# XuyangBai/PointDSC

Hardware: AMD Instinct MI355X
Metric: point-cloud pairs/sec @ N=5000 corr (higher is better)
Workload: dtype f32 (attention products as fp16x3 split (fp16 hi+lo operand pairs, three f16 MFMAs per product), f32 accumulate; fc_message / PointCN products as fp16 hi+lo split; spatial-consistency matrix stored as unorm16); 1 GPU; 3DMatch-like synthetic correspondences (BASELINE.json configs[2]): N=5000 corr, 32 pairs per step sharded over 1 GPU(s) = 32 per GPU, 12-layer PointDSC, seeded random weights; num_corr=5000, pairs_per_gpu=32, global_batch=32, compat_format=u16, layer_gemm=h3, att_leaves=canonical, latency_mode=False, range_guard=lazy (pipeline), collective=none (single process, no process group)

## Files before the change

include/pointdsc_hip.h:

```cpp
#ifndef POINTDSC_HIP_H
#define POINTDSC_HIP_H

#include <stddef.h>

#ifdef __cplusplus
extern "C" {
#endif

#define PDSC_VERSION 10
#define PDSC_CHANNELS 128
#define PDSC_MAX_K 64
#define PDSC_MAX_POWER_ITERS 32

enum pdsc_status {
    PDSC_OK = 0,
    PDSC_ERR_ARG = -1,
    PDSC_ERR_WORKSPACE = -2,
    PDSC_ERR_LAUNCH = -3
};

typedef struct pdsc_config {
    int in_dim;
    int num_layers;
    int num_channels;
// ... 92 lines not shown
    const float* part_ml;
    int nsplit, Npad;
    const float* res;
    const float* feat_in;
    float* feat_out;
    float* featB_out;
    float* qkv_out;
    void* q_split;
    void* kv_tiles;
    const void* w1; const float* b1;
    const void* w2; const float* b2;
    const void* w3; const float* b3;
    const void* wp; const float* bp;
    const void* wq; const float* bq;
    const void* wq_split;
    const void* wfrag_tail;
    const void* wfrag_head;
    int gemm_format;
    int io_flags;
    int bs, N;
    int kernel;
} pdsc_layer_call;
int pdsc_layer_run(const pdsc_layer_call* call, void* stream);

size_t    pdsc_wsplit_bytes(const pdsc_config* cfg);
long long pdsc_wsplit_offset(const pdsc_config* cfg, int section, int layer);
int       pdsc_wsplit_build(const pdsc_config* cfg, const float* wpack, void* wsplit, void* stream);
#define PDSC_WS_FRAG_TAIL 100
#define PDSC_WS_FRAG_HEAD 101
#define PDSC_WS_FRAG_TAIL_H3 102
#define PDSC_WS_FRAG_HEAD_H3 103
#define PDSC_WS_FOLD_TAIL_H3 104
#define PDSC_WS_FOLD_HEAD_H3 105
#define PDSC_WS_FOLD_W 106
size_t pdsc_wfrag_fold_tail_bytes(void);
size_t pdsc_wfrag_fold_head_bytes(void);
int pdsc_layer_prefers_block(int bs, int N);
int pdsc_layer_h3_uses_coop(int bs, int N);
size_t pdsc_wfrag_tail_bytes(void);
size_t pdsc_wfrag_head_bytes(void);
int pdsc_wfrag_build_tail(const float* w1, const float* b1, const float* w2, const float* b2, const float* w3,
                          const float* b3, void* out, int gemm_format, void* stream);
int pdsc_wfrag_build_head(const float* wp, const float* bp, const float* wq, const float* bq, void* out,
                          int gemm_format, void* stream);

size_t pdsc_attention_scratch_bytes(int bs, int N, int nsplit);
// ... 300 lines not shown
```

pointdsc_amd/_lib.py:

```python
from __future__ import annotations

import ctypes as C
import os
from pathlib import Path

PKG = Path(__file__).resolve().parent
LIB_PATH = Path(os.environ.get("POINTDSC_HIP_LIB", PKG / "libpointdsc_hip.so"))


class PointDSCLibraryError(RuntimeError):
    pass


class PdscConfig(C.Structure):
    _fields_ = [
        ("in_dim", C.c_int), ("num_layers", C.c_int), ("num_channels", C.c_int),
        ("num_iterations", C.c_int), ("k", C.c_int), ("refine_iters", C.c_int),
        ("inlier_threshold", C.c_float), ("nms_radius", C.c_float), ("refine_threshold", C.c_float),
        ("attention_precision", C.c_int), ("compat_format", C.c_int), ("layer_gemm", C.c_int),
        ("att_leaves", C.c_int), ("value_fold", C.c_int),
    ]


W_SECTIONS = [
# ... 25 lines not shown
        [("workspace", _vp), ("workspace_bytes", _sz), ("num_corr", _vp), ("num_seeds_per_pair", _vp), ("n_min", _i)] +
        [(n, _vp) for n in ("tail_stream", "fork_event", "join_event", "absmax", "range_report")])


ABI_VERSION = 10

SIGNATURES = {
    "pdsc_version": (_i, []),
    "pdsc_last_error": (C.c_char_p, []),
    "pdsc_experiments_enabled": (_i, []),
    "pdsc_wpack_floats": (_ll, [_cfgp]),
    "pdsc_wpack_offset": (_ll, [_cfgp, _i, _i]),
    "pdsc_compat_ld": (_ll, [_i]),
    "pdsc_workspace_bytes": (_sz, [_cfgp, _i, _i, _i]),
    "pdsc_workspace_offset": (_ll, [_cfgp, _i, _i, _i, C.c_char_p]),
    "pdsc_spatial_compat": (_i, [_vp, _vp, _vp, _vp, _vp, _ll, _i, _i, _vp]),
    "pdsc_spatial_compat_u16": (_i, [_vp, _vp, _vp, _vp, _ll, _i, _i, _vp]),
    "pdsc_selftest_exact_math": (_i, [_vp, _f, _vp, _vp, _ll, _vp]),
    "pdsc_selftest_mfma_valu_neighbour": (_i, [_vp, _i, _i, _vp]),
    "pdsc_classifier_hidden": (_i, [_vp, _vp, _vp, _vp, _vp, _vp, _i, _vp]),
    "pdsc_linear": (_i, [_vp, _ll, _vp, _vp, _vp, _ll, _vp, _ll, _i, _i, _i, _i, _vp]),
    "pdsc_layer0": (_i, [_vp, _i, _vp, _vp, _vp, _i, _vp]),
    "pdsc_layer_run": (_i, [C.POINTER(PdscLayerCall), _vp]),
    "pdsc_wsplit_bytes": (_sz, [_cfgp]),
    "pdsc_wsplit_offset": (_ll, [_cfgp, _i, _i]),
    "pdsc_wsplit_build": (_i, [_cfgp, _vp, _vp, _vp]),
    "pdsc_layer_prefers_block": (_i, [_i, _i]),
    "pdsc_layer_h3_uses_coop": (_i, [_i, _i]),
    "pdsc_wfrag_tail_bytes": (_sz, []),
    "pdsc_wfrag_head_bytes": (_sz, []),
    "pdsc_wfrag_fold_tail_bytes": (_sz, []),
    "pdsc_wfrag_fold_head_bytes": (_sz, []),
    "pdsc_wfrag_build_tail": (_i, [_vp] * 7 + [_i, _vp]),
    "pdsc_wfrag_build_head": (_i, [_vp] * 5 + [_i, _vp]),
    "pdsc_sc_attention_split_partials": (_i, [_vp, _vp, _vp, _i, _ll, _vp, _sz, _i, _i, _i, _i, _vp]),
    "pdsc_split_q_bytes": (_sz, [_i, _i]),
    "pdsc_split_kv_bytes": (_sz, [_i, _i]),
    "pdsc_pack_qkv_split": (_i, [_vp, _vp, _vp, _i, _i, _vp]),
    "pdsc_attention_split_scratch_bytes": (_sz, [_i, _i, _i]),
    "pdsc_attention_split_default_split": (_i, [_i, _i]),
    "pdsc_attention_leaf_count": (_i, [_i]),
    "pdsc_attention_leaf_plan": (_i, [_i, _i, _i, C.POINTER(C.c_int), C.POINTER(C.c_int)]),
    "pdsc_attention_leaf_scratch_bytes": (_sz, [_i, _i, _i]),
    "pdsc_attention_trace": (_i, [_vp]),
    "pdsc_attention_leaf_split_override": (_i, [_i]),
    "pdsc_layer_trace": (_i, [_vp]),
# ... 137 lines not shown
```

pointdsc_amd/csrc/layer.hip:

```cpp
#include <stdlib.h>
#include <type_traits>
#include "pdsc_common.h"
#include "split_layout.h"
#include "merge_partials.h"
#include "layer_args.h"
#include "layer_block.h"

namespace pdsc {

constexpr int LF_ROWS = 32;
constexpr int LF_LD = PDSC_CHANNELS + 4;
constexpr int LF_TILE = LF_ROWS * LF_LD;


#define LF_STAMP(k)                                                                                   \
    if (a.trace && lane == 0) a.trace[(((size_t)blockIdx.y * gridDim.x + blockIdx.x) * 4 + wave) * 16 + (k)] = __builtin_readcyclecounter();

template <int K>
__device__ __forceinline__ void load_w(const float* __restrict__ W, int n0, int l31, int h, f32x4 (&w)[K / 8]) {
    const float* p = W + (size_t)(n0 + l31) * K + 4 * h;
#pragma unroll
    for (int q = 0; q < K / 8; ++q) w[q] = *reinterpret_cast<const f32x4*>(p + 8 * q);
}

// ... 333 lines not shown
    using pdsc::LayerKernel;
    switch (c.kernel) {
        case PDSC_LAYER_KERNEL_BLOCK: *kernel = LayerKernel::Block; return true;
        case PDSC_LAYER_KERNEL_WAVE: *kernel = LayerKernel::Wave; return true;
        case PDSC_LAYER_KERNEL_H3: *kernel = LayerKernel::H3; return true;
        case PDSC_LAYER_KERNEL_X3: *kernel = LayerKernel::X3; return true;
        case PDSC_LAYER_KERNEL_AUTO: break;
        default: return false;
    }
    if (!a.wf_tail && !a.wf_head) {
        const char* ev = pdsc::env_str("PDSC_LAYER_VARIANT");
        const bool block = ev && (ev[0] == 'b' || ev[0] == 'w') ? ev[0] == 'b' : pdsc_layer_prefers_block(c.bs, c.N) != 0;
        *kernel = block ? LayerKernel::Block : LayerKernel::Wave;
    } else if (c.io_flags != 0) {
        *kernel = LayerKernel::H3;
    } else {
        const bool h3 = c.gemm_format == PDSC_LAYER_GEMM_H3 && pdsc::env_int("PDSC_LAYER_H3_VARIANT", 1) != 0 &&
                        pdsc::launch_layer_h3_fits(a, a.msg != nullptr || a.part_o != nullptr, a.featB_out != nullptr);
        *kernel = h3 ? LayerKernel::H3 : LayerKernel::Wave;
    }
    return true;
}

extern "C" int pdsc_layer_run(const pdsc_layer_call* call, void* stream) {
    PDSC_REQUIRE(call, "pdsc_layer_run: null call");
    const pdsc_layer_call& c = *call;
    const bool natural = c.w1 || c.b1 || c.w2 || c.b2 || c.w3 || c.b3 || c.wp || c.bp || c.wq || c.bq || c.wq_split;
    PDSC_REQUIRE(!natural || (!c.wfrag_tail && !c.wfrag_head), "pdsc_layer_run: weights given in natural layout AND as fragment streams");
    if (c.featB_out && !c.q_split && !c.kv_tiles) PDSC_REQUIRE(c.qkv_out, "pdsc_layer_run: head needs qkv_out when no split streams are given");
    pdsc::LayerArgs a = pdsc::layer_args_from_call(c);
    a.trace = c.io_flags ? nullptr : g_layer_trace;
    pdsc::LayerKernel kernel;
    PDSC_REQUIRE(choose_layer_kernel(c, a, &kernel), "pdsc_layer_run: kernel=%d", c.kernel);
    const int rc = pdsc::validate_layer_args(a, kernel, "pdsc_layer_run");
    return rc != PDSC_OK ? rc : pdsc::dispatch_layer(a, kernel, (hipStream_t)stream);
}
```

pointdsc_amd/csrc/layer_h3.hip:

```cpp
#include <stdlib.h>
#include <type_traits>
#include "pdsc_common.h"
#include "split_layout.h"
#include "merge_partials.h"
#include "layer_args.h"
#include "layer_wave.h"

namespace pdsc {

constexpr int PDSC_H3_COOP_TILES = 2560;

#define LH_STAMP(k) \
    if (TRACE && lane == 0) a.trace[(size_t)gw * 64 + (k)] = __builtin_readcyclecounter();

template <bool F = false>
constexpr int stage_tiles(int stage) { return stage == ST_FC1 || stage == ST_FC2 ? 2 : stage == ST_FC3 || stage == ST_PCN ? 4 : F ? 10 : 12; }

template <bool T, bool H, bool TRACE = false, int PIPE = 6, int EXP = 0, bool FB_PF = false, int NWV = LW_WAVES, int NBUF = 2, bool F = false>
__global__ __launch_bounds__(64 * NWV, NBUF > 2 ? 1 : 2) void layer_h3_kernel(LayerArgs a) {
    __shared__ __attribute__((aligned(16))) float Vs_all[NWV][32 * LW_VLD];
    const int lane = threadIdx.x & 63;
    const int wave = __builtin_amdgcn_readfirstlane(threadIdx.x >> 6);
    const int l31 = lane & 31, h = lane >> 5;
    const int tpp = ceil_div_dev(a.N, 32);
    const int gw = blockIdx.x * NWV + wave;
    if (gw >= a.bs * tpp) return;
    const int b = gw / tpp, tile = gw - b * tpp;
    const int m0 = b * a.N + tile * 32;
    const int valid = min(32, (a.nvalid ? a.nvalid[b] : a.N) - tile * 32);
    if (valid <= 0) return;
    const bool live = l31 < valid;
    const size_t row = (size_t)m0 + min(l31, valid - 1);
    float* Vs = Vs_all[wave];
    unsigned char* patch = reinterpret_cast<unsigned char*>(Vs);

    if (a.stagger_cycles > 0 && blockIdx.x < 512) {
        unsigned hwid;
        asm volatile("s_getreg_b32 %0, hwreg(HW_REG_HW_ID)" : "=s"(hwid));
        const bool late = a.stagger_mode == 1 ? (hwid & 1u) : a.stagger_mode == 2 ? (blockIdx.x & 1) : ((blockIdx.x >> 8) & 1);
        if (late) {
            const long long t0 = __builtin_readcyclecounter();
            while (__builtin_readcyclecounter() - t0 < a.stagger_cycles) __builtin_amdgcn_s_sleep(32);
        }
    }
    LH_STAMP(0)
    float rmax = 0.f;
    constexpr int NCH = num_chunks<T, H, F>();
    constexpr int VW = F ? LW_FOLD_VW : PDSC_CHANNELS;
    constexpr int NQ = VW / 8;
    WChunk w[NBUF];
    static_for<0, NBUF - 1>([&](auto jc) {
        constexpr int j = decltype(jc)::value;
        if constexpr (j < NCH) load_chunk<T, true, true, F>(w[j], a, j, lane);
    });

    u32x4 a0h[8], a0l[8], a1h[4], a1l[4], a2h[4], a2l[4], ayh[8], ayl[8], xqh[8], xql[8];
    f32x4 y3[16];
    if (T) {
        f32x4 x0[16];
        auto first_operand = [&](int kk) __attribute__((always_inline)) {
            if constexpr (F) {
                const float* bpr = reinterpret_cast<const float*>(a.wf_tail + LW_FOLD_BPRIME_BYTES);
#pragma unroll
                for (int u = 0; u < 2; ++u) {
                    const f32x4 bv = *reinterpret_cast<const f32x4*>(bpr + 8 * (2 * kk + u) + 4 * h);
#pragma unroll
                    for (int e = 0; e < 4; ++e) x0[2 * kk + u][e] = fmaxf(x0[2 * kk + u][e] + bv[e], 0.f);
                }
                make_kstep<true>(x0[2 * kk], x0[2 * kk + 1], a1h[kk], a1l[kk], rmax);
            } else {
                make_kstep<true>(x0[2 * kk], x0[2 * kk + 1], a0h[kk], a0l[kk], rmax);
            }
        };
        if (a.msg) {
#pragma unroll
            for (int q = 0; q < NQ; ++q) x0[q] = *reinterpret_cast<const f32x4*>(a.msg + row * VW + 8 * q + 4 * h);
#pragma unroll
// ... 17 lines not shown
                            pv[q][sp] = (EXP & 4) ? f32x4{1.f, 2.f, 3.f, (float)lane}
                                                  : *reinterpret_cast<const f32x4*>(a.part_o + e0 + (size_t)sp * a.Npad * VW + eq * (q0 + q));
#pragma unroll
                    for (int q = 0; q < GQ; ++q) {
#pragma unroll
                        for (int e = 0; e < 4; ++e) {
                            x0[q0 + q][e] = merge_apply<NS>(pv[q], mw, e);
                            asm volatile("" : "+v"(x0[q0 + q][e]));
                        }
                    }
#pragma unroll
                    for (int kk = q0 / 2; kk < (q0 + GQ) / 2; ++kk) first_operand(kk);
                    __builtin_amdgcn_sched_barrier(0);
                }
            });
        }
    } else {
#pragma unroll
        for (int q = 0; q < 16; ++q) y3[q] = *reinterpret_cast<const f32x4*>(a.feat_in + row * PDSC_CHANNELS + 8 * q + 4 * h);
#pragma unroll
        for (int kk = 0; kk < 8; ++kk) make_kstep<true>(y3[2 * kk], y3[2 * kk + 1], ayh[kk], ayl[kk], rmax);
    }
    LH_STAMP(1)

    unsigned char* img = H ? a.kv + (size_t)gw * SPL_TILE_STRIDE : nullptr;
    f32x16 acc, cross;
    f32x4 vp[4];
    u32x4 ev = {0u, 0u, 0u, 0u};
    float vt[8];

    auto epi = [&](auto stage_c, auto tile_c, auto sc, f32x4 (&v)[4]) {
        constexpr ChunkDesc d = {decltype(stage_c)::value, decltype(tile_c)::value, 0, 0};
        constexpr int s = decltype(sc)::value;
        constexpr int n0 = 32 * d.tile;
        if constexpr (d.stage == ST_FC1 || d.stage == ST_FC2) {
            if constexpr (s < 4) {
#pragma unroll
                for (int e = 0; e < 4; ++e) v[s][e] = fmaxf(v[s][e], 0.f);
                if constexpr (s & 1)
                    make_kstep<true>(v[s - 1], v[s], (d.stage == ST_FC1 ? a1h : a2h)[2 * d.tile + (s >> 1)],
                                     (d.stage == ST_FC1 ? a1l : a2l)[2 * d.tile + (s >> 1)], rmax);
            }
        } else if constexpr (d.stage == ST_FC3) {
            if constexpr (s < 4) {
#pragma unroll
                for (int e = 0; e < 4; ++e) y3[4 * d.tile + s][e] = y3[4 * d.tile + s][e] + v[s][e];
// ... 43 lines not shown
                        if constexpr (!(EXP & (2 | 8))) *reinterpret_cast<u32x4*>(dst) = ev;
                        else asm volatile("" :: "v"(ev), "v"(dst));
                    }
                    if constexpr (s >= 3 && s < 7) ev = patch_line(patch, lane, s - 3);
                } else {
                    if constexpr (s < 4) vt_put(Vs, lane, s, zero_unless(live, v[s]));
                    if constexpr (s == 3) wave_lds_sync();
                    if constexpr (s == 4 || s == 6) vt_gather(Vs, lane, (s - 4) >> 1, vt);
                    if constexpr (s == 5 || s == 7) {
                        u32x4 ch, cl;
                        vt_split(vt, ch, cl);
                        const int off = vt_offset<VW>(lane, (s - 5) >> 1, 32 * (d.tile - 8));
                        if constexpr (!(EXP & (2 | 32))) vt_store<VW>(img, off, ch, cl);
                        else asm volatile("" :: "v"(ch), "v"(cl), "v"(off));
                    }
                }
            }
        }
    };

    static_for<0, NCH>([&](auto ic) {
        constexpr int i = decltype(ic)::value;
        constexpr ChunkDesc d = chunk_desc<T, F>(i);
        if constexpr (i + NBUF - 1 < NCH && !((EXP & 1) && i >= 1)) load_chunk<T, true, true, F>(w[(i + NBUF - 1) % NBUF], a, i + NBUF - 1, lane);
        if constexpr (T && d.stage == ST_FC2 && d.tile == 0 && !(EXP & 4)) {
            const bool pf = a.io_flags & PDSC_IO_RES_PF;
            const float* r0 = a.res + (pf ? (size_t)gw * PF_TILE_FLOATS + lane * 4 : row * PDSC_CHANNELS + 4 * h);
            const int eq = pf ? 256 : 8;
#pragma unroll
            for (int q = 0; q < 16; ++q) y3[q] = *reinterpret_cast<const f32x4*>(r0 + eq * q);
        }
        const WChunk& wc = w[i % NBUF];
        if constexpr (d.chunk == 0) acc = bias_step(wc);
        constexpr bool pending = d.tile > 0;
        using StageC = std::integral_constant<int, d.stage>;
        using PrevC = std::integral_constant<int, d.tile - 1>;
        static_for<0, 4>([&](auto gc) {
            constexpr int g = decltype(gc)::value;
            if constexpr (d.stage == ST_QKV) {
                const sp16x8 wh = __builtin_bit_cast(sp16x8, wc.v[2 * g]), wl = __builtin_bit_cast(sp16x8, wc.v[2 * g + 1]);
                const sp16x8 bh = __builtin_bit_cast(sp16x8, xqh[4 * d.chunk + g]), bl = __builtin_bit_cast(sp16x8, xql[4 * d.chunk + g]);
                acc = PDSC_MFMA_X3(wl, bh, acc, 0, 0, 0);
                acc = PDSC_MFMA_X3(wh, bl, acc, 0, 0, 0);
                acc = PDSC_MFMA_X3(wh, bh, acc, 0, 0, 0);
            } else {
                const u32x4* oh = d.stage == ST_FC1 ? a0h : d.stage == ST_FC2 ? a1h : d.stage == ST_FC3 ? a2h : ayh;
                const u32x4* ol = d.stage == ST_FC1 ? a0l : d.stage == ST_FC2 ? a1l : d.stage == ST_FC3 ? a2l : ayl;
                const f32x16 zero = {0.f, 0.f, 0.f, 0.f, 0.f, 0.f, 0.f, 0.f, 0.f, 0.f, 0.f, 0.f, 0.f, 0.f, 0.f, 0.f};
                const f16x8 wh = __builtin_bit_cast(f16x8, wc.v[2 * g]), wl = __builtin_bit_cast(f16x8, wc.v[2 * g + 1]);
                const f16x8 bh = __builtin_bit_cast(f16x8, oh[4 * d.chunk + g]), bl = __builtin_bit_cast(f16x8, ol[4 * d.chunk + g]);
                cross = __builtin_amdgcn_mfma_f32_32x32x16_f16(wl, bh, (d.chunk == 0 && g == 0) ? zero : cross, 0, 0, 0);
                acc = __builtin_amdgcn_mfma_f32_32x32x16_f16(wh, bh, acc, 0, 0, 0);
                cross = __builtin_amdgcn_mfma_f32_32x32x16_f16(wh, bl, cross, 0, 0, 0);
            }
            if constexpr (pending) {
                if constexpr (d.nchunks == 2) {
                    epi(StageC{}, PrevC{}, std::integral_constant<int, 4 * d.chunk + g>{}, vp);
                } else {
                    epi(StageC{}, PrevC{}, std::integral_constant<int, 2 * g>{}, vp);
                    epi(StageC{}, PrevC{}, std::integral_constant<int, 2 * g + 1>{}, vp);
                }
            }
        });
        if constexpr (d.chunk == d.nchunks - 1) {
#pragma unroll
            for (int g = 0; g < 4; ++g)
#pragma unroll
                for (int e = 0; e < 4; ++e) vp[g][e] = d.stage != ST_QKV ? fmaf(cross[4 * g + e], H3_INV, acc[4 * g + e]) : acc[4 * g + e];
            if constexpr (d.tile == stage_tiles<F>(d.stage) - 1) {
                static_for<0, 8>([&](auto sc) { epi(StageC{}, std::integral_constant<int, d.tile>{}, sc, vp); });
            }
        }
// ... 11 lines not shown
    LH_STAMP(63)
    range_report(a.range_flag, b, rmax);
}

bool launch_layer_h3_fits(const LayerArgs& a, bool tail, bool head) {
    if (a.gemm_format != PDSC_LAYER_GEMM_H3) return false;
    if (head && (!a.qs || !a.kv || a.qkv_out)) return false;
    if (tail && head && a.feat_out) return false;
    if (tail && !head && !a.feat_out) return false;
    return a.wf_tail || !tail;
}

H3Form layer_h3_form(const LayerArgs& a, bool tail, bool head) {
    const bool fb_pf = a.io_flags & PDSC_IO_FEATB_PF;
    if (a.value_fold) {
        if (tail && head && fb_pf) return H3Form::FoldTailHeadPF;
        if (head && !tail && fb_pf) return H3Form::FoldHeadPF;
        if (tail && !head) return H3Form::FoldTail;
        set_error("pdsc_layer_run(h3): the folded layer exists with point-fragment featB only");
        return H3Form::Unserved;
    }
    if (head && fb_pf) return tail ? H3Form::TailHeadPF : H3Form::HeadPF;
    return tail && head ? H3Form::TailHead : tail ? H3Form::Tail : H3Form::Head;
}

static void h3_launch_shape(int tiles, int* nwv, int* nbuf) {
    *nwv = LW_WAVES; *nbuf = 2;
    (void)tiles;
#ifdef PDSC_EXPERIMENTS
    const int force = env_int("PDSC_LAYER_H3_SHAPE", 0);
    if (force == 42 || force == 23 || force == 13 || force == 24 || force == 14 || force == 22) { *nwv = force / 10; *nbuf = force % 10; }
#endif
}

int launch_layer_h3(const LayerArgs& a, bool tail, bool head, hipStream_t st) {
    const int waves = a.bs * ceil_div(a.N, 32);
    int nwv, nbuf;
    h3_launch_shape(waves, &nwv, &nbuf);
    if (a.value_fold) { nwv = LW_WAVES; nbuf = 2; }
    const dim3 grid(ceil_div(waves, nwv)), block(64 * nwv);
    const H3Form form = layer_h3_form(a, tail, head);
    if (form == H3Form::Unserved) return PDSC_ERR_ARG;
    const bool timed = tail && head;
    int coop_tiles = PDSC_H3_COOP_TILES;
#ifdef PDSC_EXPERIMENTS
    coop_tiles = env_int("PDSC_LAYER_H3_COOP", coop_tiles);
#endif
    if (waves <= coop_tiles && !a.trace) {
        if (timed) profile_mark_begin(PDSC_PROF_LAYER, st);
        const int rc = launch_layer_h3_coop(a, tail, head, st);
        if (timed) profile_mark_end(PDSC_PROF_LAYER, st);
        return rc;
    }
    if (timed) profile_mark_begin(PDSC_PROF_LAYER, st);
#ifdef PDSC_EXPERIMENTS
#define PDSC_H3_LAUNCH_EXTRA(TT, HH, PF)                                                                                            \
        if (nwv == 1 && nbuf == 4) hipLaunchKernelGGL((layer_h3_kernel<TT, HH, false, 6, 0, PF, 1, 4>), grid, block, 0, st, a);      \
        else if (nwv == 2 && nbuf == 3) hipLaunchKernelGGL((layer_h3_kernel<TT, HH, false, 6, 0, PF, 2, 3>), grid, block, 0, st, a); \
        else if (nwv == 1 && nbuf == 3) hipLaunchKernelGGL((layer_h3_kernel<TT, HH, false, 6, 0, PF, 1, 3>), grid, block, 0, st, a); \
        else if (nwv == 2 && nbuf == 4) hipLaunchKernelGGL((layer_h3_kernel<TT, HH, false, 6, 0, PF, 2, 4>), grid, block, 0, st, a); \
        else if (nwv == 2 && nbuf == 2) hipLaunchKernelGGL((layer_h3_kernel<TT, HH, false, 6, 0, PF, 2, 2>), grid, block, 0, st, a); \
        else
#else
#define PDSC_H3_LAUNCH_EXTRA(TT, HH, PF)
#endif
#define PDSC_H3_LAUNCH(TT, HH, PF)                                                                                                  \
    do {                                                                                                                            \
        PDSC_H3_LAUNCH_EXTRA(TT, HH, PF)                                                                                            \
        hipLaunchKernelGGL((layer_h3_kernel<TT, HH, false, 6, 0, PF>), grid, block, 0, st, a);                                       \
    } while (0)
    switch (form) {
        case H3Form::FoldTailHeadPF: hipLaunchKernelGGL((layer_h3_kernel<true, true, false, 6, 0, true, LW_WAVES, 2, true>), grid, block, 0, st, a); break;
        case H3Form::FoldHeadPF: hipLaunchKernelGGL((layer_h3_kernel<false, true, false, 6, 0, true, LW_WAVES, 2, true>), grid, block, 0, st, a); break;
        case H3Form::FoldTail: hipLaunchKernelGGL((layer_h3_kernel<true, false, false, 6, 0, false, LW_WAVES, 2, true>), grid, block, 0, st, a); break;
        case H3Form::TailHeadPF: {
#ifdef PDSC_LAYER_DIAG
            const int ex = env_int("PDSC_LAYER_H3_EXP", 0);
            if (ex == 1) hipLaunchKernelGGL((layer_h3_kernel<true, true, false, 6, 1, true>), grid, block, 0, st, a);
            else if (ex == 2) hipLaunchKernelGGL((layer_h3_kernel<true, true, false, 6, 2, true>), grid, block, 0, st, a);
            else if (ex == 4) hipLaunchKernelGGL((layer_h3_kernel<true, true, false, 6, 4, true>), grid, block, 0, st, a);
            else if (ex == 7) hipLaunchKernelGGL((layer_h3_kernel<true, true, false, 6, 7, true>), grid, block, 0, st, a);
            else if (ex == 8) hipLaunchKernelGGL((layer_h3_kernel<true, true, false, 6, 8, true>), grid, block, 0, st, a);
            else if (ex == 16) hipLaunchKernelGGL((layer_h3_kernel<true, true, false, 6, 16, true>), grid, block, 0, st, a);
            else if (ex == 32) hipLaunchKernelGGL((layer_h3_kernel<true, true, false, 6, 32, true>), grid, block, 0, st, a);
            else if (ex == 64) hipLaunchKernelGGL((layer_h3_kernel<true, true, false, 6, 64, true>), grid, block, 0, st, a);
            else
#endif
            PDSC_H3_LAUNCH(true, true, true);
            break;
        }
        case H3Form::HeadPF: PDSC_H3_LAUNCH(false, true, true); break;
        case H3Form::TailHead:
#ifdef PDSC_EXPERIMENTS
            if (a.trace) hipLaunchKernelGGL((layer_h3_kernel<true, true, true>), dim3(ceil_div(waves, LW_WAVES)), dim3(64 * LW_WAVES), 0, st, a);
            else
#endif
            PDSC_H3_LAUNCH(true, true, false);
            break;
        case H3Form::Tail: PDSC_H3_LAUNCH(true, false, false); break;
        case H3Form::Head: PDSC_H3_LAUNCH(false, true, false); break;
        case H3Form::Unserved: break;
    }
#undef PDSC_H3_LAUNCH
#undef PDSC_H3_LAUNCH_EXTRA
    if (timed) profile_mark_end(PDSC_PROF_LAYER, st);
    return check_launch("pdsc_layer_run(h3)");
}

}

using namespace pdsc;

extern "C" int pdsc_layer_h3_uses_coop(int bs, int N) {
    if (bs <= 0 || N <= 0) return 0;
    int coop_tiles = PDSC_H3_COOP_TILES;
#ifdef PDSC_EXPERIMENTS
    coop_tiles = env_int("PDSC_LAYER_H3_COOP", coop_tiles);
#endif
    return (long long)bs * ceil_div(N, 32) <= coop_tiles ? 1 : 0;
}
```

pointdsc_amd/csrc/layer_wave.h:

```cpp
#pragma once
#include <type_traits>
#include "pdsc_common.h"
#include "split_layout.h"
#include "merge_partials.h"
#include "layer_args.h"

namespace pdsc {

constexpr int LW_WAVES = 4;
constexpr int LW_VLD = 36;
constexpr int LW_QKV_BUFS = 4;
#ifndef LW_H3_BUFS
#define LW_H3_BUFS 3
#endif

struct WChunk {
    f32x4 v[8];
    float bias;
};

template <int B, int E, class F>
__device__ __forceinline__ void static_for(F&& f) {
    if constexpr (B < E) {
        f(std::integral_constant<int, B>{});
// ... 67 lines not shown
        const float* b = d.stage == ST_FC1 ? a.b1 : d.stage == ST_FC2 ? a.b2 : d.stage == ST_FC3 ? a.b3 : d.stage == ST_PCN ? a.bp : a.bq;
        const float bv = b[n];
        w.bias = h ? 0.f : bv;
    }
    switch (d.stage) {
        case ST_FC1: load_rows_f32(w, a.w1 + (size_t)n * 128 + 64 * d.chunk + 4 * h); break;
        case ST_FC2: load_rows_f32(w, a.w2 + (size_t)n * 64 + 4 * h); break;
        case ST_FC3: load_rows_f32(w, a.w3 + (size_t)n * 64 + 4 * h); break;
        case ST_PCN: load_rows_f32(w, a.wp + (size_t)n * 128 + 64 * d.chunk + 4 * h); break;
        default:
            if (X3) {
                const sp16* p = a.wq_split + (size_t)n * PDSC_CHANNELS + 64 * d.chunk + 8 * h;
#pragma unroll
                for (int k = 0; k < 4; ++k) {
                    w.v[2 * k] = *reinterpret_cast<const f32x4*>(p + 16 * k);
                    w.v[2 * k + 1] = *reinterpret_cast<const f32x4*>(p + (size_t)3 * PDSC_CHANNELS * PDSC_CHANNELS + 16 * k);
                }
            } else {
                load_rows_f32(w, a.wq + (size_t)n * 128 + 64 * d.chunk + 4 * h);
            }
    }
}

__device__ __forceinline__ void mma_f32(f32x16& acc, const WChunk& w, const f32x4* x) {
#pragma unroll
    for (int q = 0; q < 8; ++q)
#pragma unroll
        for (int e = 0; e < 4; ++e) acc = __builtin_amdgcn_mfma_f32_32x32x2f32(w.v[q][e], x[q][e], acc, 0, 0, 0);
}

__device__ __forceinline__ f32x16 bias_step(const WChunk& w) {
    const f32x16 zero = {0.f, 0.f, 0.f, 0.f, 0.f, 0.f, 0.f, 0.f, 0.f, 0.f, 0.f, 0.f, 0.f, 0.f, 0.f, 0.f};
    return __builtin_amdgcn_mfma_f32_32x32x2f32(w.bias, 1.0f, zero, 0, 0, 0);
}

__device__ __forceinline__ void mma_x3(f32x16& acc, const WChunk& w, const u32x4* xh, const u32x4* xl) {
#pragma unroll
    for (int i = 0; i < 4; ++i) {
        const sp16x8 wh = __builtin_bit_cast(sp16x8, w.v[2 * i]), wl = __builtin_bit_cast(sp16x8, w.v[2 * i + 1]);
        const sp16x8 bh = __builtin_bit_cast(sp16x8, xh[i]), bl = __builtin_bit_cast(sp16x8, xl[i]);
        acc = PDSC_MFMA_X3(wl, bh, acc, 0, 0, 0);
        acc = PDSC_MFMA_X3(wh, bl, acc, 0, 0, 0);
        acc = PDSC_MFMA_X3(wh, bh, acc, 0, 0, 0);
    }
}

__device__ __forceinline__ unsigned pack2(sp16 a, sp16 b) {
    return (unsigned)__builtin_bit_cast(unsigned short, a) | ((unsigned)__builtin_bit_cast(unsigned short, b) << 16);
}

typedef float f32x2 __attribute__((ext_vector_type(2)));

__device__ __forceinline__ void split2(float x0, float x1, unsigned& hi, unsigned& lo) { split_sp16_pair(x0, x1, hi, lo); }

__device__ __forceinline__ void split4(const f32x4& v, unsigned (&hi)[2], unsigned (&lo)[2]) {
    split2(v[0], v[1], hi[0], lo[0]);
    split2(v[2], v[3], hi[1], lo[1]);
// ... 139 lines not shown
```

pointdsc_amd/ops.py:

```python
from __future__ import annotations

import ctypes as C
from typing import Optional, Tuple

import torch

from . import _lib


def _stream() -> int:
    return torch.cuda.current_stream().cuda_stream


def _on_device(fn):
    import functools

    @functools.wraps(fn)
    def wrapped(*args, **kwargs):
        for a in list(args) + list(kwargs.values()):
            if torch.is_tensor(a) and a.is_cuda:
                with torch.cuda.device(a.device):
                    return fn(*args, **kwargs)
            if isinstance(a, (tuple, list)) and a and torch.is_tensor(a[0]) and a[0].is_cuda:
                with torch.cuda.device(a[0].device):
# ... 89 lines not shown
    w, b = _chk(w0_padded, "w0"), _chk(b0, "b0")
    y = torch.empty(x.shape[0], 128, device=x.device, dtype=torch.float32)
    _lib.check(lib.pdsc_layer0(_p(x), x.shape[1], _p(w), _p(b), _p(y), x.shape[0], _stream()), "pdsc_layer0")
    return y


LAYER_GEMMS = {"f32": 0, "h3": 1}
LAYER_KERNELS = {"auto": 0, "block": 1, "wave": 2, "h3": 3, "x3": 4}
PF_PARTIALS, PF_RES, PF_FEATB = 1, 2, 4
_TAIL_W, _HEAD_W = ("w1", "b1", "w2", "b2", "w3", "b3"), ("wp", "bp", "wq", "bq")


def pf_rows(n: int) -> int:
    return (n + 31) // 32 * 32


def _natural_weights(tail_w, head_w) -> dict:
    w = {k: _chk(t, "tail_w") for k, t in zip(_TAIL_W, tail_w or ())}
    w.update({k: _chk(t, "head_w") for k, t in zip(_HEAD_W, head_w or ())})
    return w


def _layer_run(bs: int, n: int, weights: dict, msg=None, partials=None, res=None, feat_in=None, want_feat=False, want_qkv=False,
               want_streams=True, gemm: str = "f32", io_flags: int = 0, kernel: str = "auto"):
    lib = _lib.load()
    has_tail, has_head = "w1" in weights or "wfrag_tail" in weights, "wp" in weights or "wfrag_head" in weights
    dev = next(t for t in (res, feat_in, msg) if t is not None).device
    m = bs * n

    def new(rows, cols):
        return torch.empty(rows, cols, device=dev, dtype=torch.float32)

    feat = new(m, 128) if has_tail and (want_feat or not has_head) else None
    featB = new(bs * pf_rows(n) if io_flags & PF_FEATB else m, 128) if has_head else None
    qkv = new(m, 384) if has_head and want_qkv else None
    streams = has_head and want_streams
    qs = torch.empty(int(lib.pdsc_split_q_bytes(bs, n)), device=dev, dtype=torch.uint8) if streams else None
    kv = torch.zeros(int(lib.pdsc_split_kv_bytes(bs, n)), device=dev, dtype=torch.uint8) if streams else None
    call = _lib.PdscLayerCall(bs=bs, N=n, gemm_format=LAYER_GEMMS[gemm], io_flags=io_flags, kernel=LAYER_KERNELS[kernel])
    if partials is not None:
        scratch, call.nsplit = partials
        call.Npad = (n + 255) // 256 * 256
        call.part_o = scratch.data_ptr()
        call.part_ml = scratch.data_ptr() + bs * call.nsplit * call.Npad * 128 * 4
    inputs = {k: _chk(t, k) for k, t in (("msg", msg), ("res", res), ("feat_in", feat_in)) if t is not None}
    outputs = dict(feat_out=feat, featB_out=featB, qkv_out=qkv, q_split=qs, kv_tiles=kv)
    for k, t in {**inputs, **outputs, **weights}.items():
        if t is not None:
            setattr(call, k, t.data_ptr())
    _lib.check(lib.pdsc_layer_run(C.byref(call), _stream()), "pdsc_layer_run")
    return feat, featB, qkv, qs, kv


@_on_device
def layer_fused(msg, res, feat_in, tail_w=None, head_w=None, want_feat=False):
    src = msg if msg is not None else feat_in
    return _layer_run(1, src.shape[0], _natural_weights(tail_w, head_w), msg=msg, res=res, feat_in=feat_in, want_feat=want_feat,
                      want_qkv=True, want_streams=False)[:3]


@_on_device
def sc_attention(qkv: torch.Tensor, compat: torch.Tensor, bs: int, n: int, nsplit: int = 0) -> torch.Tensor:
    lib = _lib.load()
    qkv, compat = _chk(qkv, "qkv"), _chk(compat, "compat")
    ld = compat.shape[-1]
    msg = torch.empty(bs * n, 128, device=qkv.device, dtype=torch.float32)
    nb = int(lib.pdsc_attention_scratch_bytes(bs, n, nsplit))
    scratch = torch.empty(max(nb, 16), device=qkv.device, dtype=torch.uint8)
    _lib.check(lib.pdsc_sc_attention(_p(qkv), _p(compat), ld, _p(msg), _p(scratch), nb, bs, n, nsplit, _stream()),
               "pdsc_sc_attention")
    return msg


# ... 65 lines not shown
    _lib.check(lib.pdsc_wfrag_build_tail(*[_p(_chk(w, "tail_w")) for w in tail_w], _p(out), LAYER_GEMMS[gemm], _stream()),
               "pdsc_wfrag_build_tail")
    return out


@_on_device
def frag_weights_head(head_w, gemm: str = "f32") -> torch.Tensor:
    lib = _lib.load()
    out = torch.empty(int(lib.pdsc_wfrag_head_bytes()), dtype=torch.uint8, device=head_w[0].device)
    _lib.check(lib.pdsc_wfrag_build_head(*[_p(_chk(w, "head_w")) for w in head_w], _p(out), LAYER_GEMMS[gemm], _stream()),
               "pdsc_wfrag_build_head")
    return out


def _frag_weights(tail_w, head_w, gemm: str) -> dict:
    w = {"wfrag_tail": frag_weights_tail(tail_w, gemm)} if tail_w is not None else {}
    if head_w is not None:
        w["wfrag_head"] = frag_weights_head(head_w, gemm)
    return w


@_on_device
def layer_fused_split(msg, res, feat_in, tail_w, head_w, bs: int, n: int, want_qkv: bool = False, partials=None,
                      qkv_split: bool = False, frag: bool = False, gemm: str = "f32", want_feat: bool = True):
    assert (res if res is not None else feat_in).shape[0] == bs * n
    assert head_w is not None or frag, "tail-only launches exist on fragment streams only"
    if frag:
        weights = _frag_weights(tail_w, head_w, gemm)
    else:
        assert gemm == "f32", "the H3 arithmetic exists on fragment streams only"
        weights = _natural_weights(tail_w, head_w)
        if qkv_split:
            weights["wq_split"] = split_weight(weights["wq"])
    return _layer_run(bs, n, weights, msg=msg, partials=partials, res=res, feat_in=feat_in, want_feat=want_feat, want_qkv=want_qkv,
                      gemm=gemm)


def rows_to_pf(x: torch.Tensor, bs: int, n: int) -> torch.Tensor:
    t = pf_rows(n) // 32
    x = x.reshape(bs, n, 128)
    x = torch.cat([x, x[:, -1:].expand(bs, t * 32 - n, 128)], dim=1)
    x = x.reshape(bs, t, 32, 16, 2, 4)
    return x.permute(0, 1, 3, 4, 2, 5).contiguous().reshape(-1)


def pf_to_rows(x: torch.Tensor, bs: int, rows_per_pair: int) -> torch.Tensor:
    t = rows_per_pair // 32
    x = x.reshape(bs, t, 16, 2, 32, 4)
    return x.permute(0, 1, 4, 2, 3, 5).contiguous().reshape(bs, rows_per_pair, 128)


@_on_device
def layer_fused_io(res, feat_in, tail_w, head_w, bs: int, n: int, io_flags: int, partials=None):
    feat, featB, _, qs, kv = _layer_run(bs, n, _frag_weights(tail_w, head_w, "h3"), partials=partials, res=res, feat_in=feat_in,
                                        gemm="h3", io_flags=io_flags)
    return feat, None if featB is None else featB.reshape(-1), qs, kv


# ... 476 lines not shown
```

Before: 2601 pairs/s.

## Stream H3 layer weights through an LDS ring via async global-to-LDS DMA

Replaces the register double-buffered weight-chunk loads in the H3 layer kernel with a per-wave LDS ring filled by global_load_lds_dwordx4. The loads are issued several units ahead, and each wait uses an exact vmcnt that a compile-time plan computes so it interleaves with the epilogue loads. The aim is to hide weight-fetch latency and cut VGPR pressure, at the cost of dynamic LDS per workgroup and fragile hand-counted waitcnt logic. It also adds a ragged per-pair row-count entry point (nvalid) that the H3 path accepts.

```diff
diff --git a/include/pointdsc_hip.h b/include/pointdsc_hip.h
--- a/include/pointdsc_hip.h
+++ b/include/pointdsc_hip.h
@@ -138,6 +138,7 @@
     int kernel;
 } pdsc_layer_call;
 int pdsc_layer_run(const pdsc_layer_call* call, void* stream);
+int pdsc_layer_run_ragged(const pdsc_layer_call* call, const int* num_rows, void* stream);
 
 size_t    pdsc_wsplit_bytes(const pdsc_config* cfg);
 long long pdsc_wsplit_offset(const pdsc_config* cfg, int section, int layer);
diff --git a/pointdsc_amd/_lib.py b/pointdsc_amd/_lib.py
--- a/pointdsc_amd/_lib.py
+++ b/pointdsc_amd/_lib.py
@@ -71,6 +71,7 @@
     "pdsc_linear": (_i, [_vp, _ll, _vp, _vp, _vp, _ll, _vp, _ll, _i, _i, _i, _i, _vp]),
     "pdsc_layer0": (_i, [_vp, _i, _vp, _vp, _vp, _i, _vp]),
     "pdsc_layer_run": (_i, [C.POINTER(PdscLayerCall), _vp]),
+    "pdsc_layer_run_ragged": (_i, [C.POINTER(PdscLayerCall), _vp, _vp]),
     "pdsc_wsplit_bytes": (_sz, [_cfgp]),
     "pdsc_wsplit_offset": (_ll, [_cfgp, _i, _i]),
     "pdsc_wsplit_build": (_i, [_cfgp, _vp, _vp, _vp]),
diff --git a/pointdsc_amd/csrc/layer.hip b/pointdsc_amd/csrc/layer.hip
--- a/pointdsc_amd/csrc/layer.hip
+++ b/pointdsc_amd/csrc/layer.hip
@@ -379,16 +379,25 @@
     return true;
 }
 
-extern "C" int pdsc_layer_run(const pdsc_layer_call* call, void* stream) {
-    PDSC_REQUIRE(call, "pdsc_layer_run: null call");
+static int layer_run(const pdsc_layer_call* call, const int* num_rows, void* stream, const char* who) {
+    PDSC_REQUIRE(call, "%s: null call", who);
     const pdsc_layer_call& c = *call;
     const bool natural = c.w1 || c.b1 || c.w2 || c.b2 || c.w3 || c.b3 || c.wp || c.bp || c.wq || c.bq || c.wq_split;
-    PDSC_REQUIRE(!natural || (!c.wfrag_tail && !c.wfrag_head), "pdsc_layer_run: weights given in natural layout AND as fragment streams");
-    if (c.featB_out && !c.q_split && !c.kv_tiles) PDSC_REQUIRE(c.qkv_out, "pdsc_layer_run: head needs qkv_out when no split streams are given");
+    PDSC_REQUIRE(!natural || (!c.wfrag_tail && !c.wfrag_head), "%s: weights given in natural layout AND as fragment streams", who);
+    if (c.featB_out && !c.q_split && !c.kv_tiles) PDSC_REQUIRE(c.qkv_out, "%s: head needs qkv_out when no split streams are given", who);
     pdsc::LayerArgs a = pdsc::layer_args_from_call(c);
     a.trace = c.io_flags ? nullptr : g_layer_trace;
+    a.nvalid = num_rows;
     pdsc::LayerKernel kernel;
-    PDSC_REQUIRE(choose_layer_kernel(c, a, &kernel), "pdsc_layer_run: kernel=%d", c.kernel);
-    const int rc = pdsc::validate_layer_args(a, kernel, "pdsc_layer_run");
+    PDSC_REQUIRE(choose_layer_kernel(c, a, &kernel), "%s: kernel=%d", who, c.kernel);
+    PDSC_REQUIRE(!num_rows || kernel == pdsc::LayerKernel::H3, "%s: per-pair row counts are served by the H3 kernels only", who);
+    const int rc = pdsc::validate_layer_args(a, kernel, who);
     return rc != PDSC_OK ? rc : pdsc::dispatch_layer(a, kernel, (hipStream_t)stream);
 }
+
+extern "C" int pdsc_layer_run(const pdsc_layer_call* call, void* stream) { return layer_run(call, nullptr, stream, "pdsc_layer_run"); }
+
+extern "C" int pdsc_layer_run_ragged(const pdsc_layer_call* call, const int* num_rows, void* stream) {
+    PDSC_REQUIRE(num_rows, "pdsc_layer_run_ragged: null num_rows");
+    return layer_run(call, num_rows, stream, "pdsc_layer_run_ragged");
+}
diff --git a/pointdsc_amd/csrc/layer_h3.hip b/pointdsc_amd/csrc/layer_h3.hip
--- a/pointdsc_amd/csrc/layer_h3.hip
+++ b/pointdsc_amd/csrc/layer_h3.hip
@@ -16,9 +16,51 @@
 template <bool F = false>
 constexpr int stage_tiles(int stage) { return stage == ST_FC1 || stage == ST_FC2 ? 2 : stage == ST_FC3 || stage == ST_PCN ? 4 : F ? 10 : 12; }
 
+template <bool T, bool F>
+constexpr int ring_bias_slot(int c) {
+    int n = 0;
+    for (int j = 0; j < c; ++j) n += chunk_desc<T, F>(j).chunk == 0;
+    return n % 2;
+}
+template <bool T, bool F, int U>
+__device__ __forceinline__ void ring_request(const LayerArgs& a, unsigned ring_lds, int lane) {
+    constexpr int c = U / 4, g = U % 4;
+    constexpr ChunkDesc d = chunk_desc<T, F>(c);
+    constexpr bool tail = T && c < tail_chunks<F>();
+    constexpr int idx = tail ? c : c - (T ? tail_chunks<F>() : 0);
+    constexpr int nch = tail ? tail_chunks<F>() : head_chunks<F>();
+    const unsigned char* stream = tail ? a.wf_tail : a.wf_head;
+    constexpr unsigned pos = (U % LW_RING_UNITS) * 2048;
+    ring_dma<16>(stream + idx * LW_CHUNK_BYTES + g * 2048, lane * 16, ring_lds + pos);
+    ring_dma<16>(stream + idx * LW_CHUNK_BYTES + g * 2048 + 1024, lane * 16, ring_lds + pos + 1024);
+    if constexpr (g == 0 && d.chunk == 0)
+        ring_dma<4>(stream + nch * LW_CHUNK_BYTES + tile_ordinal<F>(d) * 256, lane * 4, ring_lds + LW_RING_UNITS * 2048 + ring_bias_slot<T, F>(c) * 256);
+    asm volatile("; h3ring dma %0 end" ::"i"(U) : "memory");
+}
+template <bool T, bool F, int U>
+__device__ __forceinline__ void ring_read(f32x4* wr, float* wb, const unsigned char* ring, int lane) {
+    constexpr int c = U / 4, g = U % 4;
+    constexpr ChunkDesc d = chunk_desc<T, F>(c);
+    const unsigned char* p = ring + (U % LW_RING_UNITS) * 2048 + lane * 16;
+    wr[2 * (U % LW_RING_REGS)] = *reinterpret_cast<const f32x4*>(p);
+    wr[2 * (U % LW_RING_REGS) + 1] = *reinterpret_cast<const f32x4*>(p + 1024);
+    if constexpr (g == 0 && d.chunk == 0)
+        wb[ring_bias_slot<T, F>(c)] = *reinterpret_cast<const float*>(ring + LW_RING_UNITS * 2048 + ring_bias_slot<T, F>(c) * 256 + lane * 4);
+}
+__device__ __forceinline__ void ring_wait_lds() { asm volatile("s_waitcnt lgkmcnt(0)" ::: "memory"); }
+template <int N, int STEP>
+__device__ __forceinline__ void ring_wait_vm() {
+    static_assert(N <= 63, "vmcnt is a 6-bit counter");
+    if constexpr (N >= 0) asm volatile("s_waitcnt vmcnt(%0) ; h3ring step %1" ::"i"(N), "i"(STEP) : "memory");
+    else asm volatile("; h3ring step %0 nowait" ::"i"(STEP) : "memory");
+}
+
 template <bool T, bool H, bool TRACE = false, int PIPE = 6, int EXP = 0, bool FB_PF = false, int NWV = LW_WAVES, int NBUF = 2, bool F = false>
 __global__ __launch_bounds__(64 * NWV, NBUF > 2 ? 1 : 2) void layer_h3_kernel(LayerArgs a) {
     __shared__ __attribute__((aligned(16))) float Vs_all[NWV][32 * LW_VLD];
+    extern __shared__ __attribute__((aligned(16))) unsigned char ring_all[];
+    constexpr bool RING = NWV == LW_WAVES && NBUF == 2 && !TRACE && EXP == 0;
+    using Plan = RingPlan<T, H, FB_PF, F>;
     const int lane = threadIdx.x & 63;
     const int wave = __builtin_amdgcn_readfirstlane(threadIdx.x >> 6);
     const int l31 = lane & 31, h = lane >> 5;
@@ -48,11 +90,21 @@
     constexpr int NCH = num_chunks<T, H, F>();
     constexpr int VW = F ? LW_FOLD_VW : PDSC_CHANNELS;
     constexpr int NQ = VW / 8;
-    WChunk w[NBUF];
-    static_for<0, NBUF - 1>([&](auto jc) {
-        constexpr int j = decltype(jc)::value;
-        if constexpr (j < NCH) load_chunk<T, true, true, F>(w[j], a, j, lane);
-    });
+    WChunk w[RING ? 1 : NBUF];
+    f32x4 wr[RING ? 2 * LW_RING_REGS : 1];
+    float wb[2];
+    const unsigned char* ring = ring_all + wave * LW_RING_WAVE_BYTES;
+    const unsigned ring_lds = __builtin_amdgcn_readfirstlane(lds_offset(ring));
+    if constexpr (RING) {
+        static_for<0, LW_RING_UNITS>([&](auto uc) {
+            if constexpr (decltype(uc)::value < Plan::NST) ring_request<T, F, decltype(uc)::value>(a, ring_lds, lane);
+        });
+    } else {
+        static_for<0, NBUF - 1>([&](auto jc) {
+            constexpr int j = decltype(jc)::value;
+            if constexpr (j < NCH) load_chunk<T, true, true, F>(w[j], a, j, lane);
+        });
+    }
 
     u32x4 a0h[8], a0l[8], a1h[4], a1l[4], a2h[4], a2l[4], ayh[8], ayl[8], xqh[8], xql[8];
     f32x4 y3[16];
@@ -116,6 +168,16 @@
         for (int kk = 0; kk < 8; ++kk) make_kstep<true>(y3[2 * kk], y3[2 * kk + 1], ayh[kk], ayl[kk], rmax);
     }
     LH_STAMP(1)
+    if constexpr (RING) {
+        asm volatile("s_waitcnt vmcnt(0)" ::: "memory");
+        static_for<0, LW_RING_READ>([&](auto uc) {
+            if constexpr (decltype(uc)::value < Plan::NST) ring_read<T, F, decltype(uc)::value>(wr, wb, ring, lane);
+        });
+        ring_wait_lds();
+        static_for<LW_RING_UNITS, LW_RING_PRO_UNITS>([&](auto uc) {
+            if constexpr (decltype(uc)::value < Plan::NST) ring_request<T, F, decltype(uc)::value>(a, ring_lds, lane);
+        });
+    }
 
     unsigned char* img = H ? a.kv + (size_t)gw * SPL_TILE_STRIDE : nullptr;
     f32x16 acc, cross;
@@ -205,23 +267,36 @@
     static_for<0, NCH>([&](auto ic) {
         constexpr int i = decltype(ic)::value;
         constexpr ChunkDesc d = chunk_desc<T, F>(i);
-        if constexpr (i + NBUF - 1 < NCH && !((EXP & 1) && i >= 1)) load_chunk<T, true, true, F>(w[(i + NBUF - 1) % NBUF], a, i + NBUF - 1, lane);
-        if constexpr (T && d.stage == ST_FC2 && d.tile == 0 && !(EXP & 4)) {
+        if constexpr (!RING && i + NBUF - 1 < NCH && !((EXP & 1) && i >= 1)) load_chunk<T, true, true, F>(w[(i + NBUF - 1) % NBUF], a, i + NBUF - 1, lane);
+        auto residual_rows = [&]() __attribute__((always_inline)) {
             const bool pf = a.io_flags & PDSC_IO_RES_PF;
             const float* r0 = a.res + (pf ? (size_t)gw * PF_TILE_FLOATS + lane * 4 : row * PDSC_CHANNELS + 4 * h);
             const int eq = pf ? 256 : 8;
 #pragma unroll
             for (int q = 0; q < 16; ++q) y3[q] = *reinterpret_cast<const f32x4*>(r0 + eq * q);
-        }
-        const WChunk& wc = w[i % NBUF];
-        if constexpr (d.chunk == 0) acc = bias_step(wc);
+        };
+        const WChunk& wc = w[RING ? 0 : i % NBUF];
+        if constexpr (d.chunk == 0) {
+            if constexpr (RING) acc = bias_step(wb[ring_bias_slot<T, F>(i)]);
+            else acc = bias_step(wc);
+        }
         constexpr bool pending = d.tile > 0;
         using StageC = std::integral_constant<int, d.stage>;
         using PrevC = std::integral_constant<int, d.tile - 1>;
         static_for<0, 4>([&](auto gc) {
             constexpr int g = decltype(gc)::value;
+            if constexpr (RING) {
+                constexpr int t = 4 * i + g;
+                ring_wait_lds();
+                if constexpr (t + LW_RING_AHEAD < Plan::NST) ring_request<T, F, t + LW_RING_AHEAD>(a, ring_lds, lane);
+                ring_wait_vm<Plan::wait_count(t), t>();
+                if constexpr (t + LW_RING_READ < Plan::NST) ring_read<T, F, t + LW_RING_READ>(wr, wb, ring, lane);
+            }
+            if constexpr (g == 0 && T && d.stage == ST_FC2 && d.tile == 0 && !(EXP & 4)) residual_rows();
+            const f32x4 whv = RING ? wr[RING ? 2 * ((4 * i + g) % LW_RING_REGS) : 0] : wc.v[2 * g];
+            const f32x4 wlv = RING ? wr[RING ? 2 * ((4 * i + g) % LW_RING_REGS) + 1 : 0] : wc.v[2 * g + 1];
             if constexpr (d.stage == ST_QKV) {
-                const sp16x8 wh = __builtin_bit_cast(sp16x8, wc.v[2 * g]), wl = __builtin_bit_cast(sp16x8, wc.v[2 * g + 1]);
+                const sp16x8 wh = __builtin_bit_cast(sp16x8, whv), wl = __builtin_bit_cast(sp16x8, wlv);
                 const sp16x8 bh = __builtin_bit_cast(sp16x8, xqh[4 * d.chunk + g]), bl = __builtin_bit_cast(sp16x8, xql[4 * d.chunk + g]);
                 acc = PDSC_MFMA_X3(wl, bh, acc, 0, 0, 0);
                 acc = PDSC_MFMA_X3(wh, bl, acc, 0, 0, 0);
@@ -230,7 +305,7 @@
                 const u32x4* oh = d.stage == ST_FC1 ? a0h : d.stage == ST_FC2 ? a1h : d.stage == ST_FC3 ? a2h : ayh;
                 const u32x4* ol = d.stage == ST_FC1 ? a0l : d.stage == ST_FC2 ? a1l : d.stage == ST_FC3 ? a2l : ayl;
                 const f32x16 zero = {0.f, 0.f, 0.f, 0.f, 0.f, 0.f, 0.f, 0.f, 0.f, 0.f, 0.f, 0.f, 0.f, 0.f, 0.f, 0.f};
-                const f16x8 wh = __builtin_bit_cast(f16x8, wc.v[2 * g]), wl = __builtin_bit_cast(f16x8, wc.v[2 * g + 1]);
+                const f16x8 wh = __builtin_bit_cast(f16x8, whv), wl = __builtin_bit_cast(f16x8, wlv);
                 const f16x8 bh = __builtin_bit_cast(f16x8, oh[4 * d.chunk + g]), bl = __builtin_bit_cast(f16x8, ol[4 * d.chunk + g]);
                 cross = __builtin_amdgcn_mfma_f32_32x32x16_f16(wl, bh, (d.chunk == 0 && g == 0) ? zero : cross, 0, 0, 0);
                 acc = __builtin_amdgcn_mfma_f32_32x32x16_f16(wh, bh, acc, 0, 0, 0);
@@ -288,6 +363,16 @@
     }
     if (head && fb_pf) return tail ? H3Form::TailHeadPF : H3Form::HeadPF;
     return tail && head ? H3Form::TailHead : tail ? H3Form::Tail : H3Form::Head;
+}
+
+constexpr size_t H3_RING_LDS = (size_t)LW_WAVES * LW_RING_WAVE_BYTES;
+static_assert(sizeof(float) * LW_WAVES * 32 * LW_VLD + H3_RING_LDS <= 80 * 1024, "two workgroups per CU");
+template <class K>
+static int h3_launch_ring(K kernel, dim3 grid, dim3 block, hipStream_t st, const LayerArgs& a) {
+    const int rc = ensure_dynamic_lds(reinterpret_cast<const void*>(kernel), H3_RING_LDS, "pdsc_layer_run(h3, dynamic LDS)");
+    if (rc != PDSC_OK) return rc;
+    hipLaunchKernelGGL(kernel, grid, block, H3_RING_LDS, st, a);
+    return PDSC_OK;
 }
 
 static void h3_launch_shape(int tiles, int* nwv, int* nbuf) {
@@ -333,12 +418,13 @@
 #define PDSC_H3_LAUNCH(TT, HH, PF)                                                                                                  \
     do {                                                                                                                            \
         PDSC_H3_LAUNCH_EXTRA(TT, HH, PF)                                                                                            \
-        hipLaunchKernelGGL((layer_h3_kernel<TT, HH, false, 6, 0, PF>), grid, block, 0, st, a);                                       \
+        rc_lds = h3_launch_ring(&layer_h3_kernel<TT, HH, false, 6, 0, PF>, grid, block, st, a);                                      \
     } while (0)
+    int rc_lds = PDSC_OK;
     switch (form) {
-        case H3Form::FoldTailHeadPF: hipLaunchKernelGGL((layer_h3_kernel<true, true, false, 6, 0, true, LW_WAVES, 2, true>), grid, block, 0, st, a); break;
-        case H3Form::FoldHeadPF: hipLaunchKernelGGL((layer_h3_kernel<false, true, false, 6, 0, true, LW_WAVES, 2, true>), grid, block, 0, st, a); break;
-        case H3Form::FoldTail: hipLaunchKernelGGL((layer_h3_kernel<true, false, false, 6, 0, false, LW_WAVES, 2, true>), grid, block, 0, st, a); break;
+        case H3Form::FoldTailHeadPF: rc_lds = h3_launch_ring(&layer_h3_kernel<true, true, false, 6, 0, true, LW_WAVES, 2, true>, grid, block, st, a); break;
+        case H3Form::FoldHeadPF: rc_lds = h3_launch_ring(&layer_h3_kernel<false, true, false, 6, 0, true, LW_WAVES, 2, true>, grid, block, st, a); break;
+        case H3Form::FoldTail: rc_lds = h3_launch_ring(&layer_h3_kernel<true, false, false, 6, 0, false, LW_WAVES, 2, true>, grid, block, st, a); break;
         case H3Form::TailHeadPF: {
 #ifdef PDSC_LAYER_DIAG
             const int ex = env_int("PDSC_LAYER_H3_EXP", 0);
@@ -370,6 +456,7 @@
 #undef PDSC_H3_LAUNCH
 #undef PDSC_H3_LAUNCH_EXTRA
     if (timed) profile_mark_end(PDSC_PROF_LAYER, st);
+    if (rc_lds != PDSC_OK) return rc_lds;
     return check_launch("pdsc_layer_run(h3)");
 }
 
diff --git a/pointdsc_amd/csrc/layer_wave.h b/pointdsc_amd/csrc/layer_wave.h
--- a/pointdsc_amd/csrc/layer_wave.h
+++ b/pointdsc_amd/csrc/layer_wave.h
@@ -113,6 +113,72 @@
     }
 }
 
+#ifndef LW_RING_READ
+#define LW_RING_READ 4
+#endif
+constexpr int LW_RING_UNITS = 7;
+constexpr int LW_RING_AHEAD = LW_RING_UNITS + LW_RING_READ - 1;
+constexpr int LW_RING_REGS = 2 * LW_RING_READ;
+constexpr int LW_RING_WAVE_BYTES = LW_RING_UNITS * 2048 + 2 * 256;
+constexpr int LW_RING_PRO_UNITS = LW_RING_AHEAD;
+
+typedef __attribute__((address_space(3))) unsigned char* lds_bytes_t;
+__device__ __forceinline__ unsigned lds_offset(const void* p) { return (unsigned)(size_t)(lds_bytes_t)p; }
+
+template <int SZ>
+__device__ __forceinline__ void ring_dma(const unsigned char* base, unsigned voff, unsigned lds) {
+    unsigned keep;
+    if constexpr (SZ == 16)
+        asm volatile("s_mov_b32 %0, m0\n\ts_mov_b32 m0, %3\n\ts_nop 0\n\tglobal_load_lds_dwordx4 %1, %2\n\ts_mov_b32 m0, %0"
+                     : "=&s"(keep) : "v"(voff), "s"(base), "s"(lds) : "memory");
+    else
+        asm volatile("s_mov_b32 %0, m0\n\ts_mov_b32 m0, %3\n\ts_nop 0\n\tglobal_load_lds_dword %1, %2\n\ts_mov_b32 m0, %0"
+                     : "=&s"(keep) : "v"(voff), "s"(base), "s"(lds) : "memory");
+}
+
+template <bool H, bool FB_PF>
+constexpr int ring_epi_ops(int stage, int tile, int s) {
+    if (stage == ST_FC3) return !H && s < 4 ? 1 : 0;
+    if (stage == ST_PCN) return FB_PF ? (s < 4 ? 1 : 0) : (s >= 4 ? 1 : 0);
+    if (stage == ST_QKV) return tile < 4 ? (s >= 4 ? 1 : 0) : tile < 8 ? (s < 4 ? 1 : 0) : (s == 5 || s == 7 ? 2 : 0);
+    return 0;
+}
+
+template <bool T, bool H, bool FB_PF, bool F>
+struct RingPlan {
+    static constexpr int NCH = num_chunks<T, H, F>(), NST = 4 * NCH;
+    static constexpr int stage_last_tile(int stage) { return (stage == ST_FC1 || stage == ST_FC2 ? 2 : stage == ST_FC3 || stage == ST_PCN ? 4 : F ? 10 : 12) - 1; }
+    static constexpr int pieces(int u) { return u < 0 || u >= NST ? 0 : 2 + (u % 4 == 0 && chunk_desc<T, F>(u / 4).chunk == 0 ? 1 : 0); }
+    static constexpr int body(int t) {
+        if (t < 0 || t >= NST) return 0;
+        const ChunkDesc d = chunk_desc<T, F>(t / 4);
+        const int g = t % 4;
+        int n = 0;
+        if (T && d.stage == ST_FC2 && d.tile == 0 && g == 0) n += 16;
+        if (d.tile > 0) {
+            if (d.nchunks == 2) n += ring_epi_ops<H, FB_PF>(d.stage, d.tile - 1, 4 * d.chunk + g);
+            else n += ring_epi_ops<H, FB_PF>(d.stage, d.tile - 1, 2 * g) + ring_epi_ops<H, FB_PF>(d.stage, d.tile - 1, 2 * g + 1);
+        }
+        if (g == 3 && d.chunk == d.nchunks - 1 && d.tile == stage_last_tile(d.stage))
+            for (int s = 0; s < 8; ++s) n += ring_epi_ops<H, FB_PF>(d.stage, d.tile, s);
+        return n;
+    }
+    static constexpr int wait_count(int t) {
+        const int u = t + LW_RING_READ + 1;
+        if (u >= NST || u < LW_RING_UNITS) return -1;
+        int n = 0;
+        if (u < LW_RING_PRO_UNITS) {
+            for (int j = u + 1; j < LW_RING_PRO_UNITS; ++j) n += pieces(j);
+            for (int s = 0; s < t; ++s) n += body(s);
+            for (int s = 0; s <= t; ++s) n += pieces(s + LW_RING_AHEAD);
+        } else {
+            for (int s = t - 5; s < t; ++s) n += body(s);
+            for (int s = t - 4; s <= t; ++s) n += pieces(s + LW_RING_AHEAD);
+        }
+        return n;
+    }
+};
+
 __device__ __forceinline__ void mma_f32(f32x16& acc, const WChunk& w, const f32x4* x) {
 #pragma unroll
     for (int q = 0; q < 8; ++q)
@@ -120,10 +186,11 @@
         for (int e = 0; e < 4; ++e) acc = __builtin_amdgcn_mfma_f32_32x32x2f32(w.v[q][e], x[q][e], acc, 0, 0, 0);
 }
 
-__device__ __forceinline__ f32x16 bias_step(const WChunk& w) {
+__device__ __forceinline__ f32x16 bias_step(float bias) {
     const f32x16 zero = {0.f, 0.f, 0.f, 0.f, 0.f, 0.f, 0.f, 0.f, 0.f, 0.f, 0.f, 0.f, 0.f, 0.f, 0.f, 0.f};
-    return __builtin_amdgcn_mfma_f32_32x32x2f32(w.bias, 1.0f, zero, 0, 0, 0);
-}
+    return __builtin_amdgcn_mfma_f32_32x32x2f32(bias, 1.0f, zero, 0, 0, 0);
+}
+__device__ __forceinline__ f32x16 bias_step(const WChunk& w) { return bias_step(w.bias); }
 
 __device__ __forceinline__ void mma_x3(f32x16& acc, const WChunk& w, const u32x4* xh, const u32x4* xl) {
 #pragma unroll
diff --git a/pointdsc_amd/ops.py b/pointdsc_amd/ops.py
--- a/pointdsc_amd/ops.py
+++ b/pointdsc_amd/ops.py
@@ -135,7 +135,7 @@
 
 
 def _layer_run(bs: int, n: int, weights: dict, msg=None, partials=None, res=None, feat_in=None, want_feat=False, want_qkv=False,
-               want_streams=True, gemm: str = "f32", io_flags: int = 0, kernel: str = "auto"):
+               want_streams=True, gemm: str = "f32", io_flags: int = 0, kernel: str = "auto", num_rows=None):
     lib = _lib.load()
     has_tail, has_head = "w1" in weights or "wfrag_tail" in weights, "wp" in weights or "wfrag_head" in weights
     dev = next(t for t in (res, feat_in, msg) if t is not None).device
@@ -161,7 +161,10 @@
     for k, t in {**inputs, **outputs, **weights}.items():
         if t is not None:
             setattr(call, k, t.data_ptr())
-    _lib.check(lib.pdsc_layer_run(C.byref(call), _stream()), "pdsc_layer_run")
+    if num_rows is not None:
+        _lib.check(lib.pdsc_layer_run_ragged(C.byref(call), _p(_chk(num_rows, "num_rows", torch.int32)), _stream()), "pdsc_layer_run_ragged")
+    else:
+        _lib.check(lib.pdsc_layer_run(C.byref(call), _stream()), "pdsc_layer_run")
     return feat, featB, qkv, qs, kv
 
 
@@ -273,7 +276,7 @@
 
 @_on_device
 def layer_fused_split(msg, res, feat_in, tail_w, head_w, bs: int, n: int, want_qkv: bool = False, partials=None,
-                      qkv_split: bool = False, frag: bool = False, gemm: str = "f32", want_feat: bool = True):
+                      qkv_split: bool = False, frag: bool = False, gemm: str = "f32", want_feat: bool = True, num_rows=None):
     assert (res if res is not None else feat_in).shape[0] == bs * n
     assert head_w is not None or frag, "tail-only launches exist on fragment streams only"
     if frag:
@@ -284,7 +287,7 @@
         if qkv_split:
             weights["wq_split"] = split_weight(weights["wq"])
     return _layer_run(bs, n, weights, msg=msg, partials=partials, res=res, feat_in=feat_in, want_feat=want_feat, want_qkv=want_qkv,
-                      gemm=gemm)
+                      gemm=gemm, num_rows=num_rows)
 
 
 def rows_to_pf(x: torch.Tensor, bs: int, n: int) -> torch.Tensor:
```

Result: no change. 2590 pairs/s (-0.4%).
